# kausaltech/reina-model

Hardware: AMD Instinct MI355X
Metric: agent-days/sec (higher is better)
Workload: dtype u32

## Files before the change

### reina_model_amd/csrc/k_hospital.inc

```
#define HOSP_THREADS 1024
#define HOSP_SMALL_RANGES 32
static_assert((uint64_t)HOSP_SMALL_RANGES * 65536u >= REINA_HOSP_SMALL_AGENTS, "REINA_HOSP_RANGES of a population walked by one workgroup");

__device__ __forceinline__ int dies_in_hospital(const CAS DevParams *P, uint32_t i, uint32_t day, int sev, int v, int care) {
    if (sev == RV_FATAL) return 1;
    float p = 0.0f;
    if (sev == RV_CRITICAL) {
        if (care) return 0;
        p = P->dis.p_icu_death_no_beds[v];
    } else if (sev == RV_SEVERE) {
        if (care) return 0;
        p = P->dis.p_hospital_death_no_beds[v];
    }
    return rp_chance(p, rp_philox(P->k0, P->k1, i, day, RP_P_HOSPITAL, 0).v[0]);
}

typedef rp_sat_t SatFn;
#define SAT_NEG RP_SAT_NEG
__device__ __forceinline__ SatFn sat_then(SatFn f, SatFn g) { return rp_sat_then(f, g); }
__device__ __forceinline__ int sat_apply(SatFn f, int x) { return rp_sat_apply(f, x); }
__device__ __forceinline__ SatFn bed_fn(int type) {
    SatFn f;
    f.m = SAT_NEG;
    f.a = 0;
// ... 276 lines not shown
#endif
    const int tid = threadIdx.x;
    const uint32_t R = P->hosp_ranges, C = P->hosp_bucket_cap;
    __shared__ uint32_t s_n[HOSP_SMALL_RANGES];
    if ((uint32_t)tid < R) {
        const uint32_t c = hosp_counts(B)[tid];
        s_n[tid] = c < C ? c : C;
    }
    if (tid <= REINA_MAX_AGES) s_age_start[tid] = P->age_start[tid];
    for (int k = tid; k < HL_NR * REINA_MAX_AGES; k += HOSP_THREADS) (&s_cnt[0][0])[k] = 0;
    __syncthreads();
    if (tid == 0) {
        uint32_t acc = 0;
        for (uint32_t r = 0; r < R; r++) {
            s_base[r] = acc;
            acc += s_n[r];
        }
        s_base[R] = acc;
    }
    __syncthreads();
    const int M = (int)s_base[R];
    if (M == 0) return;
    if (tid == 0 && M > B.control[REINA_L_HOSP_PEAK]) B.control[REINA_L_HOSP_PEAK] = M;
    if (M > REINA_MAX_HOSP_EVENTS - HOSP_THREADS) {
        if (tid == 0) set_problem(B.counters, REINA_PROBLEM_HOSPITAL_OVERFLOW);
        return;
    }
    for (int p0 = tid; p0 < M; p0 += HOSP_THREADS) {
        uint32_t lo = 0, hi = R - 1;
        while (lo < hi) {
            const uint32_t mid = (lo + hi + 1) >> 1;
            if (s_base[mid] <= (uint32_t)p0) lo = mid; else hi = mid - 1;
        }
        ev[p0] = hosp_bucket(P, B, lo)[(uint32_t)p0 - s_base[lo]];
    }
    __syncthreads();
    HSTAMP(1);
    uint32_t n_max = 0;
    for (uint32_t r = 0; r < R; r++) n_max = s_n[r] > n_max ? s_n[r] : n_max;
    if (n_max <= 256u) {
        const int lane = tid & 63, wave = tid >> 6;
        for (uint32_t r = (uint32_t)wave; r < R; r += HOSP_THREADS / 64) {
            const int n = (int)s_n[r];
            uint64_t *seg = ev + s_base[r];
            if (n <= 1) continue;
            if (n <= 64) hosp_sort_wave<1>(seg, n, lane);
            else if (n <= 128) hosp_sort_wave<2>(seg, n, lane);
            else hosp_sort_wave<4>(seg, n, lane);
        }
        __syncthreads();
    } else
    for (uint32_t r0 = 0; r0 < R;) {
        uint32_t r1 = r0 + 1;
        while (r1 < R && s_base[r1 + 1] - s_base[r0] <= (uint32_t)HOSP_THREADS) r1++;
        const int n = (int)(s_base[r1] - s_base[r0]);
        if (n > HOSP_THREADS) {
            if (tid == 0) set_problem(B.counters, REINA_PROBLEM_HOSPITAL_OVERFLOW);
            return;
        }
        if (n > 1) {
            int n2 = 1;
            while (n2 < n) n2 <<= 1;
            uint64_t *seg = ev + s_base[r0];
            const int behind = (int)s_base[r0] + n + tid < M && tid < n2 - n;
            const uint64_t parked = behind ? seg[n + tid] : 0ull;
            __syncthreads();
            if (tid < n2 - n) seg[n + tid] = ~0ull;
            __syncthreads();
            hosp_sort<1>(seg, n2, tid);
            if (behind) seg[n + tid] = parked;
            __syncthreads();
        }
        r0 = r1;
    }
    HSTAMP(3);
    int b_end, c_end;
    const int b0 = B.control[REINA_L_BEDS_OPEN], c0 = B.control[REINA_L_ICU_OPEN];
    hosp_decide<HOSP_THREADS>(ev, M, b0, c0, s_f[0], s_f[1], &b_end, &c_end);
    HSTAMP(4);
// ... 5 lines not shown
        B.counters[SC_IDX(REINA_S_AVAILABLE_BEDS)] = b_end;
        B.counters[SC_IDX(REINA_S_AVAILABLE_ICU)] = c_end;
    }
    HSTAMP(6);
}

#define HOSP_P_THREADS HOSP_THREADS
#define HOSP_P_E 4
#define HOSP_WAVE_KEYS 256
static_assert(HOSP_P_THREADS * HOSP_P_E == REINA_HOSP_MAX_BUCKET_KEYS, "the workgroup network holds a full bucket");

__device__ __forceinline__ uint64_t sat_pack(SatFn fb, SatFn fc) { return rp_sat_pack(fb, fc); }
__device__ __forceinline__ void sat_unpack(uint64_t v, SatFn *fb, SatFn *fc) { rp_sat_unpack(v, fb, fc); }
__device__ __forceinline__ GAS uint64_t *hosp_agg64(const CAS DevParams *P, const GBuffers &B) {
    return B.hosp_events + HOSP_AGG_OFF(P->hosp_ranges);
}
__device__ __forceinline__ SatFn sat_id() { return rp_sat_id(); }
__device__ __forceinline__ uint64_t hosp_wait_agg(const GBuffers &B, const GAS uint64_t *agg, uint32_t q) {
    uint32_t polls = 0;
    for (;;) {
        const uint64_t v = __hip_atomic_load(&agg[q], __ATOMIC_RELAXED, __HIP_MEMORY_SCOPE_AGENT);
        if (v >> 63) return v;
        __builtin_amdgcn_s_sleep(4);
        if (++polls > (1u << 22)) {
            set_problem(B.counters, REINA_PROBLEM_SYNC_TIMEOUT);
            return 0;
        }
    }
}
__device__ __forceinline__ SatFn sat_shfl_up(SatFn f, int off) {
    SatFn r;
    r.a = __shfl_up(f.a, off);
    r.m = __shfl_up(f.m, off);
    return r;
}
__device__ __forceinline__ SatFn sat_shfl(SatFn f, int src) {
    SatFn r;
    r.a = __shfl(f.a, src);
    r.m = __shfl(f.m, src);
    return r;
}

enum { WALK_LOCAL = 0, WALK_PRESORT = 1, WALK_SHARDED = 2 };
__device__ __forceinline__ GAS uint64_t *hosp_exchange_maps(const CAS DevParams *P, const GBuffers &B, uint32_t shard) {
    return reinterpret_cast<GAS uint64_t *>(B.pressure + REINA_PRESSURE_WORDS) + (size_t)shard * P->hosp_ranges;
}
__device__ __forceinline__ GAS int32_t *hosp_prefix_table(const CAS DevParams *P, const GBuffers &B) {
// ... 346 lines not shown
```

### reina_model_amd/csrc/k_install.inc

```
enum { IL_CAND = 0, IL_ILL, IL_BOOK, IL_EV };
#ifdef REINA_NO_BYBIT
#define INSTALL_BY_BIT false
#else
#define INSTALL_BY_BIT true
#endif

__device__ __forceinline__ uint32_t install_unit_counts(const CAS DevParams *P, const GBuffers &B, int list, uint32_t first, uint32_t G, uint32_t limit,
                                                        uint32_t scan_waves, uint32_t scan_tiles, uint32_t (&c_n)[8], uint32_t (&base)[8]) {
    uint32_t tot = 0;
#pragma unroll
    for (int k = 0; k < 8; k++) {
        const uint32_t idx = first + (uint32_t)k;
        const bool in = (uint32_t)k < G && idx < limit;
        uint32_t n = 0;
        if (in) {
            if (list == IL_EV) {
                n = hosp_counts(B)[idx];
                if (n > P->hosp_bucket_cap) n = P->hosp_bucket_cap;
            } else {
                n = B.work_counts[(list == IL_CAND ? LIST_CAND : list == IL_ILL ? LIST_ILL : LIST_BOOK) * REINA_MAX_SCAN_WAVES + idx];
            }
        }
        c_n[k] = n;
        base[k] = list == IL_EV ? (in ? idx * P->hosp_bucket_cap : 0u) : scan_slice_base(in ? idx : 0u, scan_waves, scan_tiles);
// ... 37 lines not shown
    if (threadIdx.x == 0) {
        s_infectors = 0;
        s_infections = 0;
    }
    if (threadIdx.x < REINA_MAX_AGES) new_by_age[threadIdx.x] = 0;
    if (threadIdx.x < REINA_MAX_VARIANTS) new_by_variant[threadIdx.x] = 0;
    if (threadIdx.x == 0 && stage) stage->n = 0;
#ifdef REINA_INSTALL_STAMPS
    uint64_t is_t = wall_clock64();
    const int is_role = only_events ? 8 : 0;
#define ISTAMP(k) do { __syncthreads(); if (threadIdx.x == 0) { uint64_t t_ = wall_clock64(); atomicAdd((unsigned long long *)&B.mirror[is_role + (k)], (unsigned long long)(t_ - is_t)); atomicMax((unsigned long long *)&B.mirror[is_role + 4 + (k)], (unsigned long long)(t_ - is_t)); is_t = t_; } } while (0)
#else
#define ISTAMP(k) do { } while (0)
#endif
    __syncthreads();
    ISTAMP(0);
    const GAS uint4 *cand = reinterpret_cast<const GAS uint4 *>(B.candidates);
    const uint32_t lane = threadIdx.x & 63u;
    const uint32_t cap = P->max_work_items;
    const GAS uint2 *l_ill = reinterpret_cast<const GAS uint2 *>(B.work_items) + cap;
    const GAS uint2 *l_book = reinterpret_cast<const GAS uint2 *>(B.scan_lists) + cap;
    const int C_remote = (!only_events && P->n_shards > 1) ? B.control[REINA_L_CAND] : 0;
    int C_ovf = only_events ? 0 : B.control[REINA_L_CAND_OVF];
    if (C_ovf > (int)P->cand_ovf_cap) C_ovf = (int)P->cand_ovf_cap;
    const uint32_t R = P->hosp_ranges;
    uint32_t G = 8u;
    {
        const uint32_t per_slice = (uint32_t)B.control[REINA_L_CONTACTS] / (8u * (scan_waves ? scan_waves : 1u));
        if (per_slice >= 48u) G = 1u; else if (per_slice >= 24u) G = 2u; else if (per_slice >= 12u) G = 4u;
    }
    const uint32_t n_l = only_events ? 0u : (scan_waves + G - 1u) / G;
    const uint32_t n_ev = events ? (R + G - 1u) / G : 0u;
    const uint32_t n_ovf = ((uint32_t)C_ovf + 63u) / 64u, n_rem = ((uint32_t)C_remote + 63u) / 64u;
    const uint32_t total = 3u * n_l + n_ev + n_ovf + n_rem;
    const uint32_t W = (nbx * blockDim.x) >> 6, wave_g = (bx * blockDim.x + threadIdx.x) >> 6;
    const bool rotate = (W % 3u) == 0u;
    uint32_t pass = 0;
    for (uint32_t u = wave_g; u < total; u += W, pass++) {
        int list;
        uint32_t first;
        if (u < 3u * n_l) {
            list = (int)((u % 3u + (rotate ? pass : 0u)) % 3u);
            first = (u / 3u) * G;
        } else if (u < 3u * n_l + n_ev) {
            list = IL_EV;
            first = (u - 3u * n_l) * G;
        } else {
            const uint32_t f = u - 3u * n_l - n_ev;
            const bool ovf = f < n_ovf;
            const uint32_t k = (ovf ? f : f - n_ovf) * 64u + lane;
            if (k < (uint32_t)(ovf ? C_ovf : C_remote)) {
                const uint4 cd = gld(&cand[(ovf ? P->cand_ovf_base : P->max_work_items) + k]);
                if (cd.x != 0xFFFFFFFFu) {
                    const uint64_t cl = ld_claim(&B.cold[cd.x].claim);
                    const int32_t vd = B.cold[cd.x].vacc_day;
                    const uint32_t w = ld_hot(&B.hot[cd.x]);
                    if (cd.z & IMPORT_RECORD_FLAG) {
                        if (cl == rp_order_key(dp.day + 1u, 0xFFFFFu, cd.y) && RH_STATE(w) == RS_SUSCEPTIBLE)
                            install_infection(P, B, s_age_start, cd.x, w, dp.day, cd.z & 0xFFu, -1, 1, (cd.z >> 24) & 3u, new_by_age, new_by_variant, 0u, vd);
                    } else if (cl == rp_order_key(dp.day, cd.w, cd.y) && RH_STATE(w) == RS_SUSCEPTIBLE) {
                        const int32_t src = (cd.y & RP_REMOTE_SRC) ? -1 : (int32_t)cd.y;
                        install_infection(P, B, s_age_start, cd.x, w, dp.day, cd.z & 0xFFu, src, 0, dp.testing_mode, new_by_age, new_by_variant, (cd.z >> 8) & 1u, vd, false, INSTALL_BY_BIT);
                    }
                }
            }
            continue;
        }
        uint32_t c_n[8], base[8];
        const uint32_t tot = install_unit_counts(P, B, list, first, G, list == IL_EV ? R : scan_waves, scan_waves, scan_tiles, c_n, base);
        if (list == IL_CAND) {
            for (uint32_t j0 = 0; j0 < tot; j0 += 64u) {
                const uint32_t j = j0 + lane;
                if (j >= tot) continue;
                const uint4 cd = gld(&cand[install_unit_pos(j, c_n, base)]);
                const uint64_t cl = ld_claim(&B.cold[cd.x].claim);
                const int32_t vd = B.cold[cd.x].vacc_day;
                if (cl != rp_order_key(dp.day, cd.w, cd.y)) continue;
                const uint32_t w = vd >= 0 ? RH_VACCINATED : 0u;
                install_infection(P, B, s_age_start, cd.x, w, dp.day, cd.z & 0xFFu, (int32_t)cd.y, 0, dp.testing_mode, new_by_age, new_by_variant,
                                  (cd.z >> 8) & 1u, vd, false, INSTALL_BY_BIT);
            }
        } else if (list == IL_ILL) {
            for (uint32_t j0 = 0; j0 < tot; j0 += 64u) {
                const uint32_t j = j0 + lane;
                uint2 r = make_uint2(0, 0);
                if (j < tot) r = gld(&l_ill[install_unit_pos(j, c_n, base)]);
                become_ill(P, B, dp, j < tot, r.x, r.y, stage);
            }
        } else if (list == IL_BOOK) {
            for (uint32_t j0 = 0; j0 < tot; j0 += 64u) {
                const uint32_t j = j0 + lane;
                int ni = 0, cr = 0;
                if (j < tot) {
                    const uint2 r = gld(&l_book[install_unit_pos(j, c_n, base)]);
                    if (r.y == EVX_COUNT_R) {
                        cr = 1;
                        ni = B.cold[r.x].n_infected;
                    } else {
                        const int age = age_of(s_age_start, r.x, 0, (int)P->nr_ages - 1);
                        atomicAdd(&s_cnt[SL_INFECTED][age], -1);
                        if (r.y == EVX_RECOVERED_HOME) {
                            atomicAdd(&s_cnt[SL_RECOVERED][age], 1);
                        } else {
// ... 62 lines not shown
    }
    if (only_events) return;
    if (bx == 0 && threadIdx.x < REINA_MAX_AGES) {
        const int32_t v = B.control[REINA_L_DET_SIDE + threadIdx.x];
        if (v) {
            atomicAdd(&B.counters[CNT_IDX(REINA_C_DETECTED, threadIdx.x)], v);
            atomicAdd(&B.counters[CNT_IDX(REINA_C_ALL_DETECTED, threadIdx.x)], v);
            B.control[REINA_L_DET_SIDE + threadIdx.x] = 0;
        }
    }
    if (threadIdx.x == 0) {
        if (s_infectors) atomicAdd(&B.counters[SC_IDX(REINA_S_TOTAL_INFECTORS)], s_infectors);
        if (s_infections) atomicAdd(&B.counters[SC_IDX(REINA_S_TOTAL_INFECTIONS)], s_infections);
        if (bx == 0) {
            B.control[(dp.day & 1) ? REINA_L_QUEUE1 : REINA_L_QUEUE0] = 0;
            B.control[REINA_L_LEVEL1] = 0;
            B.control[REINA_L_TRACE_DONE] = 0;
            for (int q = 0; q < 4; q++) B.control[REINA_L_IMPORT_SYNC + q] = 0;
        }
    }
    ISTAMP(2);
}

enum { HI_HOSP_WG = 1, HI_INSTALL = 2, HI_EVENTS = 4 };
static_assert(HOSP_THREADS == 1024, "fused launch");
static_assert(sizeof(OnsetStage) <= (size_t)HOSP_THREADS * 4 * 8, "the stage fits the dynamic LDS of either launch shape");
DAY_KERNEL __launch_bounds__(HOSP_THREADS) void k_hosp_install(const MemberRef *M_, MemberRef one_, reina_day_t dp, uint32_t scan_waves,
                                                               uint32_t scan_tiles, int flags, uint32_t n_walk) {
    MEMBER_OF_LAUNCH;
    __shared__ int32_t s_hl[HL_NR][REINA_MAX_AGES];
    __shared__ SatFn s_f[2][HOSP_THREADS];
    extern __shared__ __align__(16) unsigned char smem_hi[];
    const bool ordered = hosp_day_is_ordered(global_buffers(mref_.B));
    uint32_t bx = blockIdx.x, nbx = gridDim.x;
    if (n_walk && ordered) {
        if (bx < n_walk) {
            hosp_walker_block(mref_, dp, s_hl, reinterpret_cast<uint64_t *>(smem_hi), s_f,
                              ((const CAS DevParams *)mref_.P)->n_shards > 1 ? WALK_SHARDED : WALK_LOCAL);
            return;
        }
        bx -= n_walk;
        nbx -= n_walk;
    }
    if (flags & HI_HOSP_WG) {
        if (bx == 0 && ordered) {
#ifdef REINA_HOSP_STAMPS
            const uint64_t hb_t = wall_clock64();
#endif
            hospital_block(mref_, dp, s_hl, s_f);
#ifdef REINA_HOSP_STAMPS
            __syncthreads();
            if (threadIdx.x == 0) {
                GAS uint64_t *mir = (GAS uint64_t *)mref_.B.mirror;
                atomicAdd((unsigned long long *)&mir[7], (unsigned long long)(wall_clock64() - hb_t));
                atomicAdd((unsigned long long *)&mir[8], 1ull);
            }
#endif
            return;
        }
        if (flags & HI_INSTALL) {
            if (bx == 0) {
                if (flags & HI_EVENTS) install_block<EXACT>(mref_, dp, scan_waves, scan_tiles, 0, 1, true, true, s_hl, nullptr);
                return;
            }
            bx--;
            nbx--;
            flags &= ~HI_EVENTS;
        }
    }
    const bool events = (flags & HI_EVENTS) && !ordered;
    if (flags & HI_INSTALL)
        install_block<EXACT>(mref_, dp, scan_waves, scan_tiles, bx, nbx, events, false, s_hl, reinterpret_cast<OnsetStage *>(smem_hi));
    else if (events)
        install_block<EXACT>(mref_, dp, scan_waves, scan_tiles, bx, nbx, true, true, s_hl, nullptr);
}

struct UploadSegs {
    uint32_t n;
    uint32_t off[8], words[8];
};
__global__ __launch_bounds__(256) void k_upload(uint32_t *d0, const uint32_t *s0, uint32_t n0, uint32_t *d1, const uint32_t *s1, UploadSegs segs) {
    const uint32_t stride = gridDim.x * blockDim.x;
    for (uint32_t k = blockIdx.x * blockDim.x + threadIdx.x; k < n0; k += stride) d0[k] = s0[k];
    for (uint32_t q = 0; q < segs.n; q++)
        for (uint32_t k = blockIdx.x * blockDim.x + threadIdx.x; k < segs.words[q]; k += stride) d1[segs.off[q] + k] = s1[segs.off[q] + k];
}

__global__ __launch_bounds__(256) void k_export(const uint4 *hist, uint32_t n_hist4, const uint4 *counters, uint32_t n_cnt4, uint4 *out) {
    const uint32_t stride = gridDim.x * blockDim.x, n = n_hist4 + n_cnt4;
    for (uint32_t k = blockIdx.x * blockDim.x + threadIdx.x; k < n; k += stride) out[k] = k < n_hist4 ? hist[k] : counters[k - n_hist4];
}
```

### reina_model_amd/csrc/k_open.inc

```
__global__ void k_init(const MemberRef *M_, int32_t beds, int32_t icu) {
    const MemberRef &mref_ = M_[blockIdx.y];
    const CAS DevParams *P = (const CAS DevParams *)mref_.P;
    const GBuffers B = global_buffers(mref_.B);
    uint32_t N = P->n_agents;
    uint32_t stride = gridDim.x * blockDim.x;
    for (uint32_t i = blockIdx.x * blockDim.x + threadIdx.x; i < N; i += stride) {
        B.hot[i] = 0;
        GAS v4u_ *rec = reinterpret_cast<GAS v4u_ *>(&B.cold[i]);
        v4u_ lo, hi;
        lo.x = 0xFFFFFFFFu; lo.y = 0xFFFFFFFFu; lo.z = 0xFFFFFFFFu; lo.w = 0u;
        hi.x = 0u; hi.y = 0xFFFFFFFFu; hi.z = 0xFFFFFFFFu; hi.w = 0xFFFFFFFFu;
        rec[0] = lo;
        rec[1] = hi;
    }
    for (size_t k = blockIdx.x * blockDim.x + threadIdx.x; k < (size_t)N * REINA_INLINE_INFECTEES; k += stride) B.infectees[k] = -1;
    for (size_t k = blockIdx.x * blockDim.x + threadIdx.x; k < REINA_BITS_WORDS(N); k += stride) B.active_bits[k] = B.infected_bits[k] = 0u;
    if (P->n_shards > 1) {
        const size_t nm = (size_t)REINA_MAX_RANGES * REINA_MAX_VARIANTS * P->mirror_slots;
        for (size_t k = blockIdx.x * blockDim.x + threadIdx.x; k < nm; k += stride) B.mirror[k] = ~0ull;
        if (blockIdx.x == 0 && threadIdx.x < REINA_MIRROR_CELLS) {
            B.mirror_meta[threadIdx.x] = P->mirror_slots < RP_MIRROR_MIN_SLOTS ? P->mirror_slots : RP_MIRROR_MIN_SLOTS;
            B.mirror_meta[REINA_MIRROR_CELLS + threadIdx.x] = 0;
        }
    }
// ... 581 lines not shown
    if (tid == 0) atomicAdd((unsigned long long *)&B.mirror[6], (unsigned long long)(wall_clock64() - ps_t));
#endif
}

__device__ __forceinline__ void weekly_imports_block(const MemberRef &mref_, const reina_day_t &dp, unsigned char *lds, uint32_t r, uint32_t W,
                                                     bool with_opening = false) {
    const CAS DevParams *P = (const CAS DevParams *)mref_.P;
    const GBuffers B = global_buffers(mref_.B);
    OpenImportsLds &OL = *reinterpret_cast<OpenImportsLds *>(lds);
    uint8_t *placed = OL.placed;
    uint32_t &s_unplaced = OL.s_unplaced, &s_import_base = OL.s_import_base;
    int32_t *new_by_age = OL.new_by_age, *new_by_variant = OL.new_by_variant, *s_age_start = OL.s_age_start;
    const int tid = threadIdx.x;
    if (tid <= REINA_MAX_AGES) s_age_start[tid] = P->age_start[tid];
    if (tid < REINA_MAX_AGES) new_by_age[tid] = 0;
    if (tid < REINA_MAX_VARIANTS) new_by_variant[tid] = 0;
    if (tid == 0) s_import_base = 0;
    __syncthreads();
#ifdef REINA_OPEN_STAMPS
    const uint64_t ws_t = wall_clock64();
#endif
    import_classes_load(P, s_age_start, &OL.classes);
    uint32_t phase = 0;
    if (with_opening) pro_imports(P, B, dp, 1, &s_import_base, placed, &s_unplaced, new_by_age, new_by_variant, s_age_start, &OL.classes, phase, false, r, W);
    pro_imports(P, B, dp, 0, &s_import_base, placed, &s_unplaced, new_by_age, new_by_variant, s_age_start, &OL.classes, phase, !with_opening, r, W);
#ifdef REINA_OPEN_STAMPS
    if (tid == 0 && r == 0) atomicAdd((unsigned long long *)&B.mirror[9], (unsigned long long)(wall_clock64() - ws_t));
#endif
}

__device__ __forceinline__ void day_imports_block(const MemberRef &mref_, const reina_day_t &dp, unsigned char *lds, uint32_t r, uint32_t W) {
    const CAS DevParams *P = (const CAS DevParams *)mref_.P;
    const GBuffers B = global_buffers(mref_.B);
    OpenImportsLds &OL = *reinterpret_cast<OpenImportsLds *>(lds);
    const int tid = threadIdx.x;
    if (tid <= REINA_MAX_AGES) OL.s_age_start[tid] = P->age_start[tid];
    if (tid == 0) OL.s_import_base = 0;
    __syncthreads();
    import_classes_load(P, OL.s_age_start, &OL.classes);
    uint32_t phase = 0;
    pro_imports(P, B, dp, 0, &OL.s_import_base, OL.placed, &OL.s_unplaced, OL.new_by_age, OL.new_by_variant, OL.s_age_start, &OL.classes,
                phase, false, r, W, true);
}

DAY_KERNEL __launch_bounds__(PRO_THREADS) void k_vaccinate(const MemberRef *M_, MemberRef one_, reina_day_t dp, uint32_t seq, VaccGeom geo) {
    MEMBER_OF_LAUNCH;
    const CAS DevParams *P = (const CAS DevParams *)mref_.P;
    const GBuffers B = global_buffers(mref_.B);
// ... 5 lines not shown
```

### reina_model_amd/csrc/k_testing.inc

```

__device__ __forceinline__ void queue_append(const CAS DevParams *P, const GBuffers &B, int which, uint32_t idx) {
    uint32_t pos = wave_alloc(&B.control[which ? REINA_L_QUEUE1 : REINA_L_QUEUE0]);
    if (pos >= P->max_queue) {
        set_problem(B.counters, REINA_PROBLEM_QUEUE_OVERFLOW);
        return;
    }
    (which ? B.queue1 : B.queue0)[pos] = idx;
}

struct OpenTraceLds;
__device__ __forceinline__ void test_detect_block(const MemberRef &mref_, const reina_day_t &dp, uint32_t bx, uint32_t nbx, unsigned char *lds) {
    const CAS DevParams *P = (const CAS DevParams *)mref_.P;
    const GBuffers B = global_buffers(mref_.B);
    int32_t *s_det = reinterpret_cast<int32_t *>(lds);
    int32_t *s_age_start = s_det + REINA_MAX_AGES;
    const int cur = dp.day & 1;
    const GAS uint32_t *q = cur ? B.queue1 : B.queue0;
    const int n = B.control[cur ? REINA_L_QUEUE1 : REINA_L_QUEUE0];
    const uint32_t ch_sh = (uint32_t)n > blockDim.x ? 6u : (uint32_t)__builtin_ctz(blockDim.x), ch = 1u << ch_sh;
    if (n <= (int)(bx * ch)) return;
    if (threadIdx.x <= REINA_MAX_AGES) s_age_start[threadIdx.x] = P->age_start[threadIdx.x];
    if (threadIdx.x < REINA_MAX_AGES) s_det[threadIdx.x] = 0;
    __syncthreads();
    for (uint32_t c = bx + nbx * (threadIdx.x >> ch_sh);; c += nbx * (blockDim.x >> ch_sh)) {
        const uint32_t k = c * ch + (threadIdx.x & (ch - 1u));
        if (c * ch >= (uint32_t)n) break;
// ... 143 lines not shown
            int32_t next, g = sib;
            if (IS_EXACT(P)) {
                g = (int32_t)B.infectee_pool[2u * (uint32_t)sib];
                next = (int32_t)B.infectee_pool[2u * (uint32_t)sib + 1u];
            } else {
                next = B.cold[sib].next_sibling;
            }
            if (!gid_local(P, g)) xsend_push(P, B, rp_gid_shard((uint32_t)g), rp_xrec(gid_index(P, g), 0u, tracer));
            else if (try_queue(P, B, gid_index(P, g), tracer, dp)) trace_accept<LEVEL>(P, B, S, nxt, gid_index(P, g));
            sib = next;
        }
        TSTAMP(3);
    }
    __syncthreads();
    {
        const uint32_t cnt = S.n < TRACE_STAGE ? S.n : TRACE_STAGE;
        if (threadIdx.x == 0 && cnt) {
            S.base_q = (uint32_t)atomicAdd(&B.control[nxt ? REINA_L_QUEUE1 : REINA_L_QUEUE0], (int)cnt);
            if (LEVEL == 0) S.base_l = (uint32_t)atomicAdd(&B.control[REINA_L_LEVEL1], (int)cnt);
        }
        __syncthreads();
        if (cnt) {
            GAS uint32_t *q = nxt ? B.queue1 : B.queue0;
            if (S.base_q + cnt > P->max_queue || (LEVEL == 0 && S.base_l + cnt > P->max_queue)) {
                if (threadIdx.x == 0) set_problem(B.counters, REINA_PROBLEM_QUEUE_OVERFLOW);
            } else {
                for (uint32_t k = threadIdx.x; k < cnt; k += blockDim.x) {
                    const uint32_t x = S.item[k];
                    q[S.base_q + k] = x;
                    if (LEVEL == 0) B.level1[S.base_l + k] = x;
                }
            }
        }
    }
    OSTAMP(LEVEL == 0 ? 1 : 4);
    if (LEVEL == 0) {
        if (threadIdx.x < REINA_MAX_AGES && s_det[threadIdx.x]) atomicAdd(&B.control[REINA_L_DET_SIDE + threadIdx.x], s_det[threadIdx.x]);
        OSTAMP(2);
    }
    if (LEVEL == 0 && FOLD == 1) {
        int &s_last = TL.s_last;
        uint32_t busy = ((uint32_t)n + ch - 1) / ch;
        if (busy > nbx) busy = nbx;
        if (busy == 1) {
            __syncthreads();
            OSTAMP(3);
            test_trace_block<1, X>(mref_, dp, 0, 1, lds);
// ... 54 lines not shown
DAY_KERNEL __launch_bounds__(256) void k_feedback(const MemberRef *M_, MemberRef one_, reina_day_t dp) {
    MEMBER_OF_LAUNCH;
    const ParamsX<true> P{(const CAS DevParams *)mref_.P};
    const GBuffers B = global_buffers(mref_.B);
    __shared__ uint32_t s_xpre[REINA_MAX_SHARDS + 1];
    xrecv_prefix(P, B, s_xpre);
    __syncthreads();
    const uint32_t total = s_xpre[P->n_shards];
    for (uint32_t idx = blockIdx.x * blockDim.x + threadIdx.x; idx < total; idx += gridDim.x * blockDim.x) {
        uint32_t from;
        const uint64_t rec = xrecv_record(P, B, s_xpre, idx, &from);
        if (rp_xrec_index(rec) < P->n_agents)
            source_gains_infectee(P, B, rp_xrec_index(rec), (int32_t)rp_xrec_gid(rec), rp_xrec_flags(rec) >> 2);
    }
    xsend_reset(P, B);
    (void)dp;
}

union OpenLds {
    OpenImportsLds imports;
    OpenTraceLds trace;
};
#define OPEN_WEEKLY_IN_STREAM 0x40000000
template <bool X>
__device__ __forceinline__ void open_role(const MemberRef &mref_, const reina_day_t &dp, uint32_t hist_slot, int weekly_own, int mode,
                                          uint32_t role, uint32_t n_roles, unsigned char *lds) {
    const bool in_stream = weekly_own == OPEN_WEEKLY_IN_STREAM;
    const uint32_t helpers = in_stream ? 0u : weekly_own > 0 ? (uint32_t)weekly_own : (uint32_t)-weekly_own;
    const uint32_t first_test = 1u + (helpers > 1u ? helpers : 1u);
    if (role == 0) {
        prologue_block(mref_, dp, hist_slot, weekly_own > 0, weekly_own < 0 ? helpers + 1u : 1u, lds);
    } else if (role < first_test) {
        if (in_stream) { }
        else if (weekly_own > 0) weekly_imports_block(mref_, dp, lds, role - 1u, helpers);
        else if (weekly_own < 0) weekly_imports_block(mref_, dp, lds, role, helpers + 1u, true);
    } else if (mode == 1) {
        test_detect_block(mref_, dp, role - first_test, n_roles - first_test, lds);
    } else if (mode == 2) {
        test_trace_block<0, X>(mref_, dp, role - first_test, n_roles - first_test, lds, 0);
    } else if (mode == 3) {
        test_trace_block<0, X>(mref_, dp, role - first_test, n_roles - first_test, lds, 1);
    }
}

DAY_KERNEL __launch_bounds__(PRO_THREADS) void k_open(const MemberRef *M_, MemberRef one_, reina_day_t dp, uint32_t hist_slot, int weekly_own, int mode,
                                                      int tickets) {
    MEMBER_OF_LAUNCH;
    __shared__ __align__(16) unsigned char s_lds[sizeof(OpenLds)];
    __shared__ uint32_t s_role;
    uint32_t role = blockIdx.x;
    if (tickets) {
        if (threadIdx.x == 0) {
            GAS int32_t *ctl = (GAS int32_t *)mref_.B.control;
            const int t = atomicAdd(&ctl[REINA_L_OPEN_TICKET], 1);
            if (t == (int)gridDim.x - 1) ctl[REINA_L_OPEN_TICKET] = 0;
            s_role = (uint32_t)t;
        }
        __syncthreads();
        role = s_role;
    }
    open_role<EXACT>(mref_, dp, hist_slot, weekly_own, mode, (uint32_t)__builtin_amdgcn_readfirstlane((int)role), gridDim.x, s_lds);
}
```

### reina_model_amd/csrc/reina_hip.hip

```cpp
#include <hip/hip_runtime.h>
#include <hip/hip_ext.h>

#if defined(__HIP_DEVICE_COMPILE__) && !defined(__gfx950__)
#error "libreina_hip is written for gfx950 (MI355X) only: build with --offload-arch=gfx950"
#endif

#include <climits>
#include <cstddef>
#include <cstdio>
#include <cstdlib>
#include <cstring>
#include <atomic>
#include <memory>
#include <mutex>
#include <string>
#include <unordered_map>
#include <vector>

#include "../../include/reina_hip.h"
#include "reina_prims.h"
#include "reina_sample.h"
#include "reina_contacts.h"

#define CNT_IDX(c, age) ((c) * REINA_MAX_AGES + (age))
// ... 328 lines not shown
    e->h_params.xchg_stride = (uint32_t)REINA_XCHG_SEG_WORDS(e->h_params.xchg_cap, e->h_params.hosp_ranges);
    if (e->h_params.hosp_ranges < 16 || e->h_params.hosp_ranges > REINA_HOSP_MAX_RANGES || (e->h_params.hosp_ranges & (e->h_params.hosp_ranges - 1))) {
        g_last_error = "hosp_ranges must be a power of two in [16, REINA_HOSP_MAX_RANGES]";
        delete e;
        return REINA_E_INVALID;
    }
    e->h_params.hosp_range_bits = 0;
    while ((1u << e->h_params.hosp_range_bits) < e->h_params.hosp_ranges) e->h_params.hosp_range_bits++;
    e->h_params.hosp_bucket_cap = REINA_HOSP_BUCKET_CAP_R(e->h_params.hosp_ranges, cfg->max_hosp_events);
    e->h_params.hosp_parallel = (cfg->n_agents > REINA_HOSP_SMALL_AGENTS || e->cfg.n_shards > 1) ? 1u : 0u;
    e->exchange_words = (uint32_t)REINA_EXCHANGE_WORDS(e->cfg.n_shards, e->h_params.hosp_ranges);
    if (e->h_params.hosp_parallel && e->h_params.hosp_bucket_cap > REINA_HOSP_MAX_BUCKET_KEYS) {
        g_last_error = "max_hosp_events too large for this population: a bucket of the event walk holds at most 4096 keys "
                       "(pass at most REINA_HOSP_MAX_EVENTS_FOR(n_agents), include/reina_hip.h)";
        delete e;
        return REINA_E_INVALID;
    }
    HIP_CHECK_OR(hipMalloc(&e->d_params, sizeof(DevParams)), free_engine(e));
    HIP_CHECK_OR(hipMalloc(&e->d_tables, sizeof(Tables)), free_engine(e));
    HIP_CHECK_OR(hipMalloc(&e->d_ref, sizeof(MemberRef)), free_engine(e));
    HIP_CHECK_OR(hipMemcpy(e->d_params, &e->h_params, sizeof(DevParams), hipMemcpyHostToDevice), free_engine(e));
    HIP_CHECK_OR(hipMemcpy(e->d_tables, &e->h_tables, sizeof(Tables), hipMemcpyHostToDevice), free_engine(e));
    const size_t walk_lds = (size_t)HOSP_P_THREADS * HOSP_P_E * 8, small_lds = (size_t)REINA_MAX_HOSP_EVENTS * 8;
    const int day_lds = (int)day_shared_bytes(REINA_LDS_ROWS, REINA_LDS_CROWS, REINA_MAX_SHARDS), inst_lds = (int)(walk_lds > small_lds ? walk_lds : small_lds);
#define SET_LDS(kernel, bytes)                                                                                                                       \
    HIP_CHECK_OR(hipFuncSetAttribute(reinterpret_cast<const void *>(kernel<false, false>), hipFuncAttributeMaxDynamicSharedMemorySize, bytes), free_engine(e)); \
    HIP_CHECK_OR(hipFuncSetAttribute(reinterpret_cast<const void *>(kernel<true, false>), hipFuncAttributeMaxDynamicSharedMemorySize, bytes), free_engine(e));  \
    HIP_CHECK_OR(hipFuncSetAttribute(reinterpret_cast<const void *>(kernel<false, true>), hipFuncAttributeMaxDynamicSharedMemorySize, bytes), free_engine(e))
#define SET_LDS_DAY(SP)                                                                                                                              \
    HIP_CHECK_OR(hipFuncSetAttribute(reinterpret_cast<const void *>(k_day<false, false, SP>), hipFuncAttributeMaxDynamicSharedMemorySize, day_lds), free_engine(e)); \
    HIP_CHECK_OR(hipFuncSetAttribute(reinterpret_cast<const void *>(k_day<true, false, SP>), hipFuncAttributeMaxDynamicSharedMemorySize, day_lds), free_engine(e));  \
    HIP_CHECK_OR(hipFuncSetAttribute(reinterpret_cast<const void *>(k_day<false, true, SP>), hipFuncAttributeMaxDynamicSharedMemorySize, day_lds), free_engine(e))
    SET_LDS_DAY(false);
    SET_LDS_DAY(true);
#undef SET_LDS_DAY
    {
        const void *day_kernels[6] = {reinterpret_cast<const void *>(k_day<false, false, false>), reinterpret_cast<const void *>(k_day<false, false, true>),
                                      reinterpret_cast<const void *>(k_day<true, false, false>), reinterpret_cast<const void *>(k_day<true, false, true>),
                                      reinterpret_cast<const void *>(k_day<false, true, false>), reinterpret_cast<const void *>(k_day<false, true, true>)};
        for (const void *k : day_kernels) {
            hipFuncAttributes fa;
            HIP_CHECK_OR(hipFuncGetAttributes(&fa, k), free_engine(e));
            if (fa.numRegs != 128 || fa.localSizeBytes != 0) {
                g_last_error = "k_day was built with " + std::to_string(fa.numRegs) + " VGPRs / " + std::to_string(fa.localSizeBytes) +
                               " bytes of scratch: it names v104..v127 by hand and needs 128 / 0 (rebuild with the ROCm release the sources were written for)";
                free_engine(e);
                return REINA_E_HIP;
            }
        }
    }
    SET_LDS(k_hosp_presort, (int)walk_lds);
    SET_LDS(k_hosp_install, inst_lds);
#undef SET_LDS
    {
        hipFuncAttributes fa;
        HIP_CHECK_OR(hipFuncGetAttributes(&fa, reinterpret_cast<const void *>(k_small_days)), free_engine(e));
        e->small_static_lds = fa.sharedSizeBytes;
        const size_t most = 160u * 1024u > fa.sharedSizeBytes ? 160u * 1024u - fa.sharedSizeBytes : 0u;
        HIP_CHECK_OR(hipFuncSetAttribute(reinterpret_cast<const void *>(k_small_days), hipFuncAttributeMaxDynamicSharedMemorySize, (int)most), free_engine(e));
        HIP_CHECK_OR(hipMalloc(&e->d_bar, 256), free_engine(e));
        HIP_CHECK_OR(hipMemset(e->d_bar, 0, 256), free_engine(e));
        HIP_CHECK_OR(hipMalloc(&e->d_days, sizeof(SmallDayRec) * SMALL_MAX_DAYS), free_engine(e));
    }
    e->counted_live = true;
    g_live_engines++;
    *out = e;
    return REINA_OK;
}

int reina_destroy(reina_engine_t *e) {
    if (!e) return REINA_E_INVALID;
    free_engine(e);
    return REINA_OK;
}

// ... 248 lines not shown
        const uint32_t cap = K > 1 ? (e->n_cus / K > 0 ? e->n_cus / K : 1u) : e->n_cus;
        if (day_blocks + stream_imports > cap && cap > stream_imports) day_blocks = cap - stream_imports;
        weekly_own = OPEN_WEEKLY_IN_STREAM;
    }
    g->weekly_own = weekly_own;
    g->stream_imports = stream_imports;
    g->day_blocks = day_blocks;
    g->xtrace = e->exact && dp.testing_mode == RT_ALL_WITH_SYMPTOMS_CT;
    return REINA_OK;
}

static int launch_day_open(reina_engine_t *e, const MemberRef *refs, uint32_t K, const reina_day_t &dp, uint32_t hist_slot, hipStream_t s) {
    DayGeom geo;
    if (int rc = day_geometry(e, K, dp, &geo)) return rc;
    const uint32_t N = e->cfg.n_agents;
    const int today = profiled_kind(e, dp.day);
    const int weekly_own = geo.weekly_own;
    int tg = grid_for(N / 64 + 1, PRO_THREADS, 64);
    if (K > 1 && tg > (int)(e->n_cus / K)) tg = e->n_cus / K > 0 ? (int)(e->n_cus / K) : 1;
    const bool ct = dp.testing_mode == RT_ALL_WITH_SYMPTOMS_CT;
    const int helpers = weekly_own == OPEN_WEEKLY_IN_STREAM ? 0 : weekly_own > 0 ? weekly_own : -weekly_own;
    const int g0 = 1 + (helpers > 1 ? helpers : 1), g = g0 + tg;
    const int open_tickets = (K > 1 || g > (int)e->n_cus || e->open_tickets || N <= 8000000u) ? 1 : 0;
    if (!e->testing_ever) {
        LAUNCH_DAY(e, today, REINA_PK_OPEN, k_open, dim3(g0, K), dim3(PRO_THREADS), 0, s, dp, hist_slot, weekly_own, 0, open_tickets);
    } else if (ct && N <= 8000000u && !geo.xtrace) {
        LAUNCH_DAY(e, today, REINA_PK_OPEN, k_open, dim3(g, K), dim3(PRO_THREADS), 0, s, dp, hist_slot, weekly_own, 3, open_tickets);
    } else if (ct) {
        LAUNCH_DAY(e, today, REINA_PK_OPEN, k_open, dim3(g, K), dim3(PRO_THREADS), 0, s, dp, hist_slot, weekly_own, 2, open_tickets);
        if (!geo.xtrace) LAUNCH_DAY(e, today, REINA_PK_TRACE1, k_test_trace1, dim3(grid_for(N / 64 + 1, 256, 256), K), dim3(256), 0, s, dp);
    } else {
        LAUNCH_DAY(e, today, REINA_PK_OPEN, k_open, dim3(g, K), dim3(PRO_THREADS), 0, s, dp, hist_slot, weekly_own, 1, open_tickets);
    }
    HIP_CHECK(hipGetLastError());
    return REINA_OK;
}

static int xchg_grid(const reina_engine_t *e) { return grid_for(e->cfg.xchg_cap * (e->cfg.n_shards - 1u) / 4u + 1u, 256, 128); }

static int launch_day_trace(reina_engine_t *e, const MemberRef *refs, uint32_t K, const reina_day_t &dp, hipStream_t s) {
    DayGeom geo;
    if (int rc = day_geometry(e, K, dp, &geo)) return rc;
    if (!geo.xtrace) return REINA_OK;
    const int today = profiled_kind(e, dp.day);
    LAUNCH_DAY(e, today, REINA_PK_XCHG, k_xtrace, dim3(xchg_grid(e), K), dim3(256), 0, s, dp, 0);
    LAUNCH_DAY(e, today, REINA_PK_TRACE1, k_test_trace1, dim3(grid_for(e->cfg.n_agents / 64 + 1, 256, 256), K), dim3(256), 0, s, dp);
    HIP_CHECK(hipGetLastError());
    return REINA_OK;
}

static int launch_day_main(reina_engine_t *e, const MemberRef *refs, uint32_t K, const reina_day_t &dp, hipStream_t s) {
    DayGeom geo;
    if (int rc = day_geometry(e, K, dp, &geo)) return rc;
    const int today = profiled_kind(e, dp.day);
    if (geo.xtrace) LAUNCH_DAY(e, today, REINA_PK_XCHG, k_xtrace, dim3(xchg_grid(e), K), dim3(256), 0, s, dp, 1);
    const uint32_t day_blocks = geo.day_blocks, stream_imports = geo.stream_imports;
// ... 78 lines not shown
    const int today = profiled_kind(e, dp.day);
    const bool sharded = e->cfg.n_shards > 1;
    if (sharded)
        LAUNCH_DAY(e, today, REINA_PK_REMOTE, k_remote, dim3(grid_for(N / 256 + 1, 256, 256), K), dim3(256), 0, s, dp);
    {
        const uint32_t scan_tiles = ((N >> 2) + 127u) / 128u;
        const uint32_t scan_waves = e->cur_scan_waves;
        int ig = grid_for(N / 64 + 1, HOSP_THREADS, 128) * 2;
        {
            const uint32_t units = 3u * ((scan_waves + 7u) / 8u) + (e->h_params.hosp_ranges + 7u) / 8u;
            const int want = (int)((units + HOSP_THREADS / 64 - 1) / (HOSP_THREADS / 64));
            if (want > ig) ig = want;
            if (ig > (int)e->n_cus) ig = (int)e->n_cus;
        }
        if (K > 1 && ig > (int)(128 / K)) ig = (int)(128 / K) >= 2 ? ((int)(128 / K) & ~1) : 1;
        const bool par = e->h_params.hosp_parallel != 0;
        if (par) {
            const uint32_t n_walk = (e->h_params.hosp_ranges + e->walk_div - 1u) / e->walk_div;
            int rest = (int)e->n_cus - (int)n_walk;
            if (K > 1) rest = (int)(e->n_cus / K) - (int)n_walk;
            if (rest > ig) rest = ig;
            if (rest < 2) rest = 2;
            LAUNCH_DAY(e, today, REINA_PK_INSTALL, k_hosp_install, dim3(n_walk + rest, K), dim3(HOSP_THREADS),
                         (size_t)HOSP_P_THREADS * HOSP_P_E * 8, s, dp, scan_waves, scan_tiles, HI_INSTALL | HI_EVENTS, n_walk);
        } else {
            if (ig < 2 && K == 1) ig = 2;
            LAUNCH_DAY(e, today, REINA_PK_INSTALL, k_hosp_install, dim3(ig + 1, K), dim3(HOSP_THREADS), (size_t)REINA_MAX_HOSP_EVENTS * 8, s, dp, scan_waves, scan_tiles, HI_HOSP_WG | HI_INSTALL | HI_EVENTS, 0u);
        }
    }
    HIP_CHECK(hipGetLastError());
    return REINA_OK;
}

static bool small_days_engine_ok(const reina_engine_t *e) {
    if (!e->fused_day || e->cfg.n_shards != 1 || e->exact || e->coll_fn || e->h_params.hosp_parallel != 0u) return false;
    if (e->cfg.n_agents > REINA_HOSP_SMALL_AGENTS) return false;
    if (e->day_mode != 0 || e->open_tickets || e->imports_in_open) return false;
    if ((uint32_t)g_live_engines.load() * e->small_wgs > e->n_cus) return false;
    return SMALL_TAIL_BYTES + e->small_static_lds <= 160u * 1024u;
}
static bool small_day_record(reina_engine_t *e, const reina_day_t &dp, SmallDayRec *rec) {
    if (dp.n_vaccinations != 0u) return false;
    DayGeom geo;
    if (day_geometry(e, 1, dp, &geo) != REINA_OK) return false;
    const uint32_t W = e->small_wgs;
    const uint32_t helpers = geo.weekly_own == OPEN_WEEKLY_IN_STREAM ? 0u : geo.weekly_own > 0 ? (uint32_t)geo.weekly_own : (uint32_t)-geo.weekly_own;
    if (W < 1u + (helpers > 1u ? helpers : 1u) + 1u || geo.stream_imports > 1u) return false;
    std::memset(rec, 0, sizeof(*rec));
    rec->dp = dp;
    rec->weekly_own = geo.weekly_own;
// ... 436 lines not shown
```

Measured before the change: 46.47 billion.

## Specialize open and hospital-install kernels by mode; unify flat candidate install path

Splits k_hosp_install into a walker/install kernel and a separate hospital-workgroup kernel. It also templates k_open on its mode so the runtime mode branches are resolved at compile time. The flat remote/overflow candidate path is folded into the shared per-lane install loop instead of a separate inline block, and overflow checks get __builtin_expect hints. The goal is to cut divergent branches, register pressure and dynamic LDS per launch shape. The cost is more kernel instantiations and a larger code footprint.

```diff
diff --git a/reina_model_amd/csrc/k_hospital.inc b/reina_model_amd/csrc/k_hospital.inc
--- a/reina_model_amd/csrc/k_hospital.inc
+++ b/reina_model_amd/csrc/k_hospital.inc
@@ -322,7 +322,7 @@
     const int M = (int)s_base[R];
     if (M == 0) return;
     if (tid == 0 && M > B.control[REINA_L_HOSP_PEAK]) B.control[REINA_L_HOSP_PEAK] = M;
-    if (M > REINA_MAX_HOSP_EVENTS - HOSP_THREADS) {
+    if (__builtin_expect(M > REINA_MAX_HOSP_EVENTS - HOSP_THREADS, 0)) {
         if (tid == 0) set_problem(B.counters, REINA_PROBLEM_HOSPITAL_OVERFLOW);
         return;
     }
@@ -354,7 +354,7 @@
         uint32_t r1 = r0 + 1;
         while (r1 < R && s_base[r1 + 1] - s_base[r0] <= (uint32_t)HOSP_THREADS) r1++;
         const int n = (int)(s_base[r1] - s_base[r0]);
-        if (n > HOSP_THREADS) {
+        if (__builtin_expect(n > HOSP_THREADS, 0)) {
             if (tid == 0) set_problem(B.counters, REINA_PROBLEM_HOSPITAL_OVERFLOW);
             return;
         }
@@ -406,7 +406,7 @@
         const uint64_t v = __hip_atomic_load(&agg[q], __ATOMIC_RELAXED, __HIP_MEMORY_SCOPE_AGENT);
         if (v >> 63) return v;
         __builtin_amdgcn_s_sleep(4);
-        if (++polls > (1u << 22)) {
+        if (__builtin_expect(++polls > (1u << 22), 0)) {
             set_problem(B.counters, REINA_PROBLEM_SYNC_TIMEOUT);
             return 0;
         }
diff --git a/reina_model_amd/csrc/k_install.inc b/reina_model_amd/csrc/k_install.inc
--- a/reina_model_amd/csrc/k_install.inc
+++ b/reina_model_amd/csrc/k_install.inc
@@ -83,7 +83,7 @@
     const GAS uint2 *l_book = reinterpret_cast<const GAS uint2 *>(B.scan_lists) + cap;
     const int C_remote = (!only_events && P->n_shards > 1) ? B.control[REINA_L_CAND] : 0;
     int C_ovf = only_events ? 0 : B.control[REINA_L_CAND_OVF];
-    if (C_ovf > (int)P->cand_ovf_cap) C_ovf = (int)P->cand_ovf_cap;
+    if (__builtin_expect(C_ovf > (int)P->cand_ovf_cap, 0)) C_ovf = (int)P->cand_ovf_cap;
     const uint32_t R = P->hosp_ranges;
     uint32_t G = 8u;
     {
@@ -99,47 +99,56 @@
     uint32_t pass = 0;
     for (uint32_t u = wave_g; u < total; u += W, pass++) {
         int list;
-        uint32_t first;
-        if (u < 3u * n_l) {
+        uint32_t first = 0u;
+        const bool flat = !only_events && u >= 3u * n_l + n_ev;
+        uint32_t flat_base = 0u, flat_n = 0u;
+        if (!only_events && u < 3u * n_l) {
             list = (int)((u % 3u + (rotate ? pass : 0u)) % 3u);
             first = (u / 3u) * G;
-        } else if (u < 3u * n_l + n_ev) {
+        } else if (!flat) {
             list = IL_EV;
             first = (u - 3u * n_l) * G;
         } else {
             const uint32_t f = u - 3u * n_l - n_ev;
             const bool ovf = f < n_ovf;
-            const uint32_t k = (ovf ? f : f - n_ovf) * 64u + lane;
-            if (k < (uint32_t)(ovf ? C_ovf : C_remote)) {
-                const uint4 cd = gld(&cand[(ovf ? P->cand_ovf_base : P->max_work_items) + k]);
-                if (cd.x != 0xFFFFFFFFu) {
-                    const uint64_t cl = ld_claim(&B.cold[cd.x].claim);
-                    const int32_t vd = B.cold[cd.x].vacc_day;
-                    const uint32_t w = ld_hot(&B.hot[cd.x]);
-                    if (cd.z & IMPORT_RECORD_FLAG) {
-                        if (cl == rp_order_key(dp.day + 1u, 0xFFFFFu, cd.y) && RH_STATE(w) == RS_SUSCEPTIBLE)
-                            install_infection(P, B, s_age_start, cd.x, w, dp.day, cd.z & 0xFFu, -1, 1, (cd.z >> 24) & 3u, new_by_age, new_by_variant, 0u, vd);
-                    } else if (cl == rp_order_key(dp.day, cd.w, cd.y) && RH_STATE(w) == RS_SUSCEPTIBLE) {
-                        const int32_t src = (cd.y & RP_REMOTE_SRC) ? -1 : (int32_t)cd.y;
-                        install_infection(P, B, s_age_start, cd.x, w, dp.day, cd.z & 0xFFu, src, 0, dp.testing_mode, new_by_age, new_by_variant, (cd.z >> 8) & 1u, vd, false, INSTALL_BY_BIT);
-                    }
-                }
-            }
-            continue;
-        }
-        uint32_t c_n[8], base[8];
-        const uint32_t tot = install_unit_counts(P, B, list, first, G, list == IL_EV ? R : scan_waves, scan_waves, scan_tiles, c_n, base);
+            const uint32_t k0 = (ovf ? f : f - n_ovf) * 64u, n = (uint32_t)(ovf ? C_ovf : C_remote);
+            list = IL_CAND;
+            flat_base = (ovf ? P->cand_ovf_base : P->max_work_items) + k0;
+            flat_n = n > k0 ? (n - k0 < 64u ? n - k0 : 64u) : 0u;
+        }
+        uint32_t c_n[8] = {0u, 0u, 0u, 0u, 0u, 0u, 0u, 0u}, base[8] = {0u, 0u, 0u, 0u, 0u, 0u, 0u, 0u};
+        const uint32_t tot = flat ? flat_n : install_unit_counts(P, B, list, first, G, list == IL_EV ? R : scan_waves, scan_waves, scan_tiles, c_n, base);
         if (list == IL_CAND) {
             for (uint32_t j0 = 0; j0 < tot; j0 += 64u) {
                 const uint32_t j = j0 + lane;
                 if (j >= tot) continue;
-                const uint4 cd = gld(&cand[install_unit_pos(j, c_n, base)]);
+                const uint4 cd = gld(&cand[flat ? flat_base + j : install_unit_pos(j, c_n, base)]);
+                if (__builtin_expect(flat && cd.x == 0xFFFFFFFFu, 0)) continue;
                 const uint64_t cl = ld_claim(&B.cold[cd.x].claim);
                 const int32_t vd = B.cold[cd.x].vacc_day;
-                if (cl != rp_order_key(dp.day, cd.w, cd.y)) continue;
-                const uint32_t w = vd >= 0 ? RH_VACCINATED : 0u;
-                install_infection(P, B, s_age_start, cd.x, w, dp.day, cd.z & 0xFFu, (int32_t)cd.y, 0, dp.testing_mode, new_by_age, new_by_variant,
-                                  (cd.z >> 8) & 1u, vd, false, INSTALL_BY_BIT);
+                uint32_t w, tmode = dp.testing_mode, has_list = (cd.z >> 8) & 1u;
+                int32_t src = (int32_t)cd.y;
+                int imp = 0;
+                bool by_bit = INSTALL_BY_BIT;
+                if (flat) {
+                    w = ld_hot(&B.hot[cd.x]);
+                    if (cd.z & IMPORT_RECORD_FLAG) {
+                        if (cl != rp_order_key(dp.day + 1u, 0xFFFFFu, cd.y)) continue;
+                        src = -1;
+                        imp = 1;
+                        tmode = (cd.z >> 24) & 3u;
+                        has_list = 0u;
+                        by_bit = false;
+                    } else {
+                        if (cl != rp_order_key(dp.day, cd.w, cd.y)) continue;
+                        if (cd.y & RP_REMOTE_SRC) src = -1;
+                    }
+                    if (RH_STATE(w) != RS_SUSCEPTIBLE) continue;
+                } else {
+                    if (cl != rp_order_key(dp.day, cd.w, cd.y)) continue;
+                    w = vd >= 0 ? RH_VACCINATED : 0u;
+                }
+                install_infection(P, B, s_age_start, cd.x, w, dp.day, cd.z & 0xFFu, src, imp, tmode, new_by_age, new_by_variant, has_list, vd, false, by_bit);
             }
         } else if (list == IL_ILL) {
             for (uint32_t j0 = 0; j0 < tot; j0 += 64u) {
@@ -248,18 +257,17 @@
     ISTAMP(2);
 }
 
-enum { HI_HOSP_WG = 1, HI_INSTALL = 2, HI_EVENTS = 4 };
 static_assert(HOSP_THREADS == 1024, "fused launch");
 static_assert(sizeof(OnsetStage) <= (size_t)HOSP_THREADS * 4 * 8, "the stage fits the dynamic LDS of either launch shape");
 DAY_KERNEL __launch_bounds__(HOSP_THREADS) void k_hosp_install(const MemberRef *M_, MemberRef one_, reina_day_t dp, uint32_t scan_waves,
-                                                               uint32_t scan_tiles, int flags, uint32_t n_walk) {
+                                                               uint32_t scan_tiles, uint32_t n_walk) {
     MEMBER_OF_LAUNCH;
     __shared__ int32_t s_hl[HL_NR][REINA_MAX_AGES];
     __shared__ SatFn s_f[2][HOSP_THREADS];
     extern __shared__ __align__(16) unsigned char smem_hi[];
     const bool ordered = hosp_day_is_ordered(global_buffers(mref_.B));
     uint32_t bx = blockIdx.x, nbx = gridDim.x;
-    if (n_walk && ordered) {
+    if (ordered) {
         if (bx < n_walk) {
             hosp_walker_block(mref_, dp, s_hl, reinterpret_cast<uint64_t *>(smem_hi), s_f,
                               ((const CAS DevParams *)mref_.P)->n_shards > 1 ? WALK_SHARDED : WALK_LOCAL);
@@ -268,8 +276,18 @@
         bx -= n_walk;
         nbx -= n_walk;
     }
-    if (flags & HI_HOSP_WG) {
-        if (bx == 0 && ordered) {
+    install_block<EXACT>(mref_, dp, scan_waves, scan_tiles, bx, nbx, !ordered, false, s_hl, reinterpret_cast<OnsetStage *>(smem_hi));
+}
+
+template <bool GROUP>
+__global__ __launch_bounds__(HOSP_THREADS) void k_hospwg_install(const MemberRef *M_, MemberRef one_, reina_day_t dp, uint32_t scan_waves,
+                                                                 uint32_t scan_tiles) {
+    MEMBER_OF_LAUNCH;
+    __shared__ int32_t s_hl[HL_NR][REINA_MAX_AGES];
+    __shared__ SatFn s_f[2][HOSP_THREADS];
+    extern __shared__ __align__(16) unsigned char smem_hi[];
+    if (blockIdx.x == 0) {
+        if (hosp_day_is_ordered(global_buffers(mref_.B))) {
 #ifdef REINA_HOSP_STAMPS
             const uint64_t hb_t = wall_clock64();
 #endif
@@ -282,23 +300,12 @@
                 atomicAdd((unsigned long long *)&mir[8], 1ull);
             }
 #endif
-            return;
-        }
-        if (flags & HI_INSTALL) {
-            if (bx == 0) {
-                if (flags & HI_EVENTS) install_block<EXACT>(mref_, dp, scan_waves, scan_tiles, 0, 1, true, true, s_hl, nullptr);
-                return;
-            }
-            bx--;
-            nbx--;
-            flags &= ~HI_EVENTS;
-        }
-    }
-    const bool events = (flags & HI_EVENTS) && !ordered;
-    if (flags & HI_INSTALL)
-        install_block<EXACT>(mref_, dp, scan_waves, scan_tiles, bx, nbx, events, false, s_hl, reinterpret_cast<OnsetStage *>(smem_hi));
-    else if (events)
-        install_block<EXACT>(mref_, dp, scan_waves, scan_tiles, bx, nbx, true, true, s_hl, nullptr);
+        } else {
+            install_block<false>(mref_, dp, scan_waves, scan_tiles, 0, 1, true, true, s_hl, nullptr);
+        }
+        return;
+    }
+    install_block<false>(mref_, dp, scan_waves, scan_tiles, blockIdx.x - 1u, gridDim.x - 1u, false, false, s_hl, reinterpret_cast<OnsetStage *>(smem_hi));
 }
 
 struct UploadSegs {
diff --git a/reina_model_amd/csrc/k_open.inc b/reina_model_amd/csrc/k_open.inc
--- a/reina_model_amd/csrc/k_open.inc
+++ b/reina_model_amd/csrc/k_open.inc
@@ -627,8 +627,9 @@
 #endif
     import_classes_load(P, s_age_start, &OL.classes);
     uint32_t phase = 0;
-    if (with_opening) pro_imports(P, B, dp, 1, &s_import_base, placed, &s_unplaced, new_by_age, new_by_variant, s_age_start, &OL.classes, phase, false, r, W);
-    pro_imports(P, B, dp, 0, &s_import_base, placed, &s_unplaced, new_by_age, new_by_variant, s_age_start, &OL.classes, phase, !with_opening, r, W);
+#pragma nounroll
+    for (int pre_init = with_opening ? 1 : 0; pre_init >= 0; pre_init--)
+        pro_imports(P, B, dp, pre_init, &s_import_base, placed, &s_unplaced, new_by_age, new_by_variant, s_age_start, &OL.classes, phase, !with_opening, r, W);
 #ifdef REINA_OPEN_STAMPS
     if (tid == 0 && r == 0) atomicAdd((unsigned long long *)&B.mirror[9], (unsigned long long)(wall_clock64() - ws_t));
 #endif
diff --git a/reina_model_amd/csrc/k_testing.inc b/reina_model_amd/csrc/k_testing.inc
--- a/reina_model_amd/csrc/k_testing.inc
+++ b/reina_model_amd/csrc/k_testing.inc
@@ -1,7 +1,7 @@
 
 __device__ __forceinline__ void queue_append(const CAS DevParams *P, const GBuffers &B, int which, uint32_t idx) {
     uint32_t pos = wave_alloc(&B.control[which ? REINA_L_QUEUE1 : REINA_L_QUEUE0]);
-    if (pos >= P->max_queue) {
+    if (__builtin_expect(pos >= P->max_queue, 0)) {
         set_problem(B.counters, REINA_PROBLEM_QUEUE_OVERFLOW);
         return;
     }
@@ -191,7 +191,7 @@
         __syncthreads();
         if (cnt) {
             GAS uint32_t *q = nxt ? B.queue1 : B.queue0;
-            if (S.base_q + cnt > P->max_queue || (LEVEL == 0 && S.base_l + cnt > P->max_queue)) {
+            if (__builtin_expect(S.base_q + cnt > P->max_queue || (LEVEL == 0 && S.base_l + cnt > P->max_queue), 0)) {
                 if (threadIdx.x == 0) set_problem(B.counters, REINA_PROBLEM_QUEUE_OVERFLOW);
             } else {
                 for (uint32_t k = threadIdx.x; k < cnt; k += blockDim.x) {
@@ -292,18 +292,18 @@
     OpenTraceLds trace;
 };
 #define OPEN_WEEKLY_IN_STREAM 0x40000000
-template <bool X>
-__device__ __forceinline__ void open_role(const MemberRef &mref_, const reina_day_t &dp, uint32_t hist_slot, int weekly_own, int mode,
+template <bool X, int MODE = -1>
+__device__ __forceinline__ void open_role(const MemberRef &mref_, const reina_day_t &dp, uint32_t hist_slot, int weekly_own, int mode_rt,
                                           uint32_t role, uint32_t n_roles, unsigned char *lds) {
+    const int mode = MODE >= 0 ? MODE : mode_rt;
     const bool in_stream = weekly_own == OPEN_WEEKLY_IN_STREAM;
     const uint32_t helpers = in_stream ? 0u : weekly_own > 0 ? (uint32_t)weekly_own : (uint32_t)-weekly_own;
     const uint32_t first_test = 1u + (helpers > 1u ? helpers : 1u);
     if (role == 0) {
         prologue_block(mref_, dp, hist_slot, weekly_own > 0, weekly_own < 0 ? helpers + 1u : 1u, lds);
     } else if (role < first_test) {
-        if (in_stream) { }
-        else if (weekly_own > 0) weekly_imports_block(mref_, dp, lds, role - 1u, helpers);
-        else if (weekly_own < 0) weekly_imports_block(mref_, dp, lds, role, helpers + 1u, true);
+        const bool with_opening = weekly_own < 0;
+        if (!in_stream && weekly_own != 0) weekly_imports_block(mref_, dp, lds, with_opening ? role : role - 1u, with_opening ? helpers + 1u : helpers, with_opening);
     } else if (mode == 1) {
         test_detect_block(mref_, dp, role - first_test, n_roles - first_test, lds);
     } else if (mode == 2) {
@@ -313,8 +313,8 @@
     }
 }
 
-DAY_KERNEL __launch_bounds__(PRO_THREADS) void k_open(const MemberRef *M_, MemberRef one_, reina_day_t dp, uint32_t hist_slot, int weekly_own, int mode,
-                                                      int tickets) {
+template <bool GROUP, bool EXACT, int MODE>
+__global__ __launch_bounds__(PRO_THREADS) void k_open(const MemberRef *M_, MemberRef one_, reina_day_t dp, uint32_t hist_slot, int weekly_own, int tickets) {
     MEMBER_OF_LAUNCH;
     __shared__ __align__(16) unsigned char s_lds[sizeof(OpenLds)];
     __shared__ uint32_t s_role;
@@ -329,5 +329,5 @@
         __syncthreads();
         role = s_role;
     }
-    open_role<EXACT>(mref_, dp, hist_slot, weekly_own, mode, (uint32_t)__builtin_amdgcn_readfirstlane((int)role), gridDim.x, s_lds);
-}
+    open_role<EXACT, MODE>(mref_, dp, hist_slot, weekly_own, MODE, (uint32_t)__builtin_amdgcn_readfirstlane((int)role), gridDim.x, s_lds);
+}
diff --git a/reina_model_amd/csrc/reina_hip.hip b/reina_model_amd/csrc/reina_hip.hip
--- a/reina_model_amd/csrc/reina_hip.hip
+++ b/reina_model_amd/csrc/reina_hip.hip
@@ -374,7 +374,7 @@
     HIP_CHECK_OR(hipMemcpy(e->d_params, &e->h_params, sizeof(DevParams), hipMemcpyHostToDevice), free_engine(e));
     HIP_CHECK_OR(hipMemcpy(e->d_tables, &e->h_tables, sizeof(Tables), hipMemcpyHostToDevice), free_engine(e));
     const size_t walk_lds = (size_t)HOSP_P_THREADS * HOSP_P_E * 8, small_lds = (size_t)REINA_MAX_HOSP_EVENTS * 8;
-    const int day_lds = (int)day_shared_bytes(REINA_LDS_ROWS, REINA_LDS_CROWS, REINA_MAX_SHARDS), inst_lds = (int)(walk_lds > small_lds ? walk_lds : small_lds);
+    const int day_lds = (int)day_shared_bytes(REINA_LDS_ROWS, REINA_LDS_CROWS, REINA_MAX_SHARDS);
 #define SET_LDS(kernel, bytes)                                                                                                                       \
     HIP_CHECK_OR(hipFuncSetAttribute(reinterpret_cast<const void *>(kernel<false, false>), hipFuncAttributeMaxDynamicSharedMemorySize, bytes), free_engine(e)); \
     HIP_CHECK_OR(hipFuncSetAttribute(reinterpret_cast<const void *>(kernel<true, false>), hipFuncAttributeMaxDynamicSharedMemorySize, bytes), free_engine(e));  \
@@ -402,7 +402,9 @@
         }
     }
     SET_LDS(k_hosp_presort, (int)walk_lds);
-    SET_LDS(k_hosp_install, inst_lds);
+    SET_LDS(k_hosp_install, (int)walk_lds);
+    HIP_CHECK_OR(hipFuncSetAttribute(reinterpret_cast<const void *>(k_hospwg_install<false>), hipFuncAttributeMaxDynamicSharedMemorySize, (int)small_lds), free_engine(e));
+    HIP_CHECK_OR(hipFuncSetAttribute(reinterpret_cast<const void *>(k_hospwg_install<true>), hipFuncAttributeMaxDynamicSharedMemorySize, (int)small_lds), free_engine(e));
 #undef SET_LDS
     {
         hipFuncAttributes fa;
@@ -697,16 +699,23 @@
     const int helpers = weekly_own == OPEN_WEEKLY_IN_STREAM ? 0 : weekly_own > 0 ? weekly_own : -weekly_own;
     const int g0 = 1 + (helpers > 1 ? helpers : 1), g = g0 + tg;
     const int open_tickets = (K > 1 || g > (int)e->n_cus || e->open_tickets || N <= 8000000u) ? 1 : 0;
+#define K_OPEN(MODE, GRID)                                                                                                                               \
+    do {                                                                                                                                                 \
+        if (K > 1) LAUNCH_TIMED(e, today, REINA_PK_OPEN, (k_open<true, false, MODE>), dim3(GRID, K), dim3(PRO_THREADS), 0, s, refs, e->h_ref, dp, hist_slot, weekly_own, open_tickets); \
+        else if (MODE != 3 && e->exact) LAUNCH_TIMED(e, today, REINA_PK_OPEN, (k_open<false, MODE != 3, MODE>), dim3(GRID, K), dim3(PRO_THREADS), 0, s, refs, e->h_ref, dp, hist_slot, weekly_own, open_tickets); \
+        else LAUNCH_TIMED(e, today, REINA_PK_OPEN, (k_open<false, false, MODE>), dim3(GRID, K), dim3(PRO_THREADS), 0, s, refs, e->h_ref, dp, hist_slot, weekly_own, open_tickets); \
+    } while (0)
     if (!e->testing_ever) {
-        LAUNCH_DAY(e, today, REINA_PK_OPEN, k_open, dim3(g0, K), dim3(PRO_THREADS), 0, s, dp, hist_slot, weekly_own, 0, open_tickets);
+        K_OPEN(0, g0);
     } else if (ct && N <= 8000000u && !geo.xtrace) {
-        LAUNCH_DAY(e, today, REINA_PK_OPEN, k_open, dim3(g, K), dim3(PRO_THREADS), 0, s, dp, hist_slot, weekly_own, 3, open_tickets);
+        K_OPEN(3, g);
     } else if (ct) {
-        LAUNCH_DAY(e, today, REINA_PK_OPEN, k_open, dim3(g, K), dim3(PRO_THREADS), 0, s, dp, hist_slot, weekly_own, 2, open_tickets);
+        K_OPEN(2, g);
         if (!geo.xtrace) LAUNCH_DAY(e, today, REINA_PK_TRACE1, k_test_trace1, dim3(grid_for(N / 64 + 1, 256, 256), K), dim3(256), 0, s, dp);
     } else {
-        LAUNCH_DAY(e, today, REINA_PK_OPEN, k_open, dim3(g, K), dim3(PRO_THREADS), 0, s, dp, hist_slot, weekly_own, 1, open_tickets);
-    }
+        K_OPEN(1, g);
+    }
+#undef K_OPEN
     HIP_CHECK(hipGetLastError());
     return REINA_OK;
 }
@@ -831,10 +840,11 @@
             if (rest > ig) rest = ig;
             if (rest < 2) rest = 2;
             LAUNCH_DAY(e, today, REINA_PK_INSTALL, k_hosp_install, dim3(n_walk + rest, K), dim3(HOSP_THREADS),
-                         (size_t)HOSP_P_THREADS * HOSP_P_E * 8, s, dp, scan_waves, scan_tiles, HI_INSTALL | HI_EVENTS, n_walk);
+                         (size_t)HOSP_P_THREADS * HOSP_P_E * 8, s, dp, scan_waves, scan_tiles, n_walk);
         } else {
             if (ig < 2 && K == 1) ig = 2;
-            LAUNCH_DAY(e, today, REINA_PK_INSTALL, k_hosp_install, dim3(ig + 1, K), dim3(HOSP_THREADS), (size_t)REINA_MAX_HOSP_EVENTS * 8, s, dp, scan_waves, scan_tiles, HI_HOSP_WG | HI_INSTALL | HI_EVENTS, 0u);
+            if (K > 1) LAUNCH_TIMED(e, today, REINA_PK_INSTALL, (k_hospwg_install<true>), dim3(ig + 1, K), dim3(HOSP_THREADS), (size_t)REINA_MAX_HOSP_EVENTS * 8, s, refs, e->h_ref, dp, scan_waves, scan_tiles);
+            else LAUNCH_TIMED(e, today, REINA_PK_INSTALL, (k_hospwg_install<false>), dim3(ig + 1, K), dim3(HOSP_THREADS), (size_t)REINA_MAX_HOSP_EVENTS * 8, s, refs, e->h_ref, dp, scan_waves, scan_tiles);
         }
     }
     HIP_CHECK(hipGetLastError());
```

Measured after the change: 42.54 billion. 0.915x the previous value.
